# JackShDr/InfluentialRS

Hardware: AMD Instinct MI355X
Metric: scored user-item pairs/sec (whole node) (higher is better)
Workload: dtype f32; 1 GPU; c2: n_item=3415, d=128, L=200, H=4, layers=6, ffn=256; one greedy path-search step; users_per_gpu=4096, top_k=100, sweep=bf16 filter + exact f32 re-score, parallelism=single GPU

## Files before the change

influentialrs_amd/csrc/decoder.hip:

```cpp
#include "irs_internal.h"

typedef __attribute__((ext_vector_type(16))) float f32x16;

__global__ void __launch_bounds__(256) k_embed(const int64_t *__restrict__ seq, const float *__restrict__ E,
                                               const float *__restrict__ pe, float *__restrict__ x, int rows, int L,
                                               int d, float sqrtd, int64_t n_item) {
    int row = blockIdx.x * 4 + (threadIdx.x >> 6);
    int lane = threadIdx.x & 63;
    if (row >= rows) return;
    int64_t id = seq[row];
    if (id < 0) id = 0;
    if (id > n_item) id = n_item;
    int t = row % L;
    const float *e = E + id * (int64_t)d;
    const float *p = pe + (int64_t)t * d;
    float *o = x + (int64_t)row * d;
    for (int c = lane; c < d; c += 64) o[c] = __fadd_rn(__fmul_rn(e[c], sqrtd), p[c]);
}

__global__ void k_pif(const int64_t *__restrict__ user, const float *__restrict__ U, const float *__restrict__ w,
                      const float *__restrict__ b, float *__restrict__ r_u, int B, int ud, int64_t n_user) {
    int i = blockIdx.x * blockDim.x + threadIdx.x;
    if (i >= B) return;
    int64_t u = user[i];
// ... 1450 lines not shown
__device__ __forceinline__ x6_u32x4 x6_rd_sync(unsigned int base) {
    x6_u32x4 v;
    asm volatile("ds_read_b128 %0, %1 offset:%2\n\ts_waitcnt lgkmcnt(0)" : "=v"(v) : "v"(base), "i"(OFF));
    return v;
}

struct SeqTarget {
    int seq;
    float k[8], v[8];
};
__device__ __forceinline__ unsigned int seq_diag_mask(int L, int qb, bool tgt, int pq) {
    unsigned int pm = 0;
    const int k0_ = 16 * qb;
    if (L <= k0_) return 0;
    if (L - k0_ < 16) pm = (0xFFFFu << (L - k0_)) & 0xFFFFu;
    if (tgt && L - 1 >= k0_ && L - 1 < k0_ + 16) pm |= 1u << (L - 1 - k0_);
    if (pq >= k0_ && pq < k0_ + 16) pm |= 1u << (pq - k0_);
    return pm;
}
__device__ __forceinline__ void seq_attn_block(const float *Ks, const char *Vp, int PL, int L, int qb, unsigned int pm_diag, float tgt_add,
                                               bool tgt_ok, int pq, const float *qscr, float4 *of, bool store, int seq, SeqTarget &tg);
#define SEQ_KQ_SCALE 1.0f
#ifndef SEQ_ASM_DMA
#define SEQ_ASM_DMA 1
#endif
#ifndef SEQ_EXP
#define SEQ_EXP 0
#endif
#ifndef SEQ_IDLE_SKIP
#define SEQ_IDLE_SKIP 1
#endif
#ifndef SEQ_FRONT_RIDE
#define SEQ_FRONT_RIDE 1
#endif
#define X6_SEQ_VECS (256 + 12 * 32 * 4 + 384)
#define X6_SEQ_KIMG (3 * 16384 + X6_SEQ_VECS * 4)
#define X6_SEQ_VIMG (X6_SEQ_KIMG + 32768)
#define X6_SEQ_SCR (X6_SEQ_VIMG + 32768)
#define X6_SEQ_SCR_B 4608
__host__ __device__ constexpr int x6_seq_lds_bytes() { return X6_SEQ_SCR + 8 * X6_SEQ_SCR_B; }
#ifdef X6_STAMP
#define X6_T(v_) { unsigned long long t_; asm volatile("s_memtime %0\n\ts_waitcnt lgkmcnt(0)" : "=s"(t_) :: "memory"); v_ = t_; }
#if X6_STAMP + 0 == 2
#define X6_TI(v_)
#else
#define X6_TI(v_) X6_T(v_)
#endif
#define X6_PH(i_) { unsigned long long t_; asm volatile("s_memtime %0\n\ts_waitcnt lgkmcnt(0)" : "=s"(t_) :: "memory"); st_ph[i_] += t_ - st_prev; st_prev = t_; }
#else
#define X6_T(v_)
#define X6_TI(v_)
#define X6_PH(i_)
#endif
template <int QP0, int NW, bool EMBED, int NT = 4, int NPL = 3, bool SEQ = false>
__global__ void __launch_bounds__(64 * NW, (NT == 8 || NW == 8) ? 1 : 2) k_block_x6(BlockX6Args a) {
    static_assert(!SEQ || (NT == 4 && NPL == 2 && NW == 8 && !EMBED && QP0 == 3), "the sequence-resident form: d = 128, float16 planes, eight waves, no q | k | v tail");
    constexpr int NP = 8 * NPL, STEP_B = x6_step_b(NPL);
    using x6_plane = typename std::conditional<NPL == 2, x6_f16x8, x6_bf16x8>::type;
    constexpr int D = 32 * NT, F = 256, NSLOT = SEQ ? 3 : x6_nslot(NPL), LEAD = NSLOT - 1, PPW = NP / NW, HT = NT / 4;
    constexpr int NFRONT = SEQ ? 3 * NT : 0;
    constexpr float WS = x6_wscale(NPL), IWS = 1.0f / WS;
    constexpr bool RESID_LATE = X6_RESID_LATE && NPL == 2 && NT == 4 && !EMBED && NSLOT == 4 && (NW == 4 || NW == 8);
    constexpr bool RESID_SEP = RESID_LATE || SEQ;
    constexpr int NLOAD = 4 * NT;
    constexpr int NPRE = x6_npre(NT), NOUT = NT * HT;
    constexpr int S0 = EMBED ? NPRE : 0;
// ... 95 lines not shown
            for (int i = tid; i < D; i += 64 * NW) {
                vecs[V_B2 + i] = a.b2[i];
                vecs[V_G + i] = a.g[i];
                vecs[V_B + i] = a.b[i];
                vecs[V_O + 0 * D + i] = a.bo ? a.bo[i] : 0.f;
                vecs[V_O + 1 * D + i] = a.g1[i];
                vecs[V_O + 2 * D + i] = a.b1n[i];
                vecs[V_O + 3 * D + i] = a.c ? a.c[i] : 0.f;
                vecs[V_O + 4 * D + i] = a.c ? a.g2[i] : 0.f;
                vecs[V_O + 5 * D + i] = a.c ? a.b2n[i] : 0.f;
            }
        }
    }
#ifdef X6_STAGGER
    if (blockIdx.x >= 256 && blockIdx.x < 512)
        for (int i = 0; i < X6_STAGGER; ++i) __builtin_amdgcn_s_sleep(127);
#endif
    int mtile = SEQ ? (int)blockIdx.x * NW + wave : (m0 >> 5) + wave;
    const bool l_h1 = li >= 16;
    const int l_b = l_h1 ? sh_b[1] : sh_b[0];
    const int s_j = l_b >= 0 ? 16 * (l_h1 ? sh_qb[1] : sh_qb[0]) + (li & 15) : 0x3FFFFFFF;
    const int l_row0 = l_h1 ? sh_row0[1] : sh_row0[0];
    const int mt = SEQ ? 0x7FFFFFFF : m0 + wave * 32 + li;
    size_t fbase = (size_t)mtile * (4 * NT) * 64 + lane;
    const unsigned int lds0 = (unsigned int)(size_t)(__attribute__((address_space(3))) char *)smem;
    unsigned int fr_addr = lds0 + lane * 16;
    unsigned int vecs_addr = lds0 + NSLOT * STEP_B + 16 * lk;
    constexpr int qoff = NOUT * QP0;
    constexpr int nsteps_c = NFRONT + x6_nstep(NT) - qoff;
    constexpr int SEQ_LSTEPS = NFRONT + NPRE + 1;
    static_assert(!SEQ || SEQ_LSTEPS % NSLOT == 0, "slot numbering repeats per layer");
    int ly = 0, nsteps_rt = nsteps_c;
    bool last_rt = true;
#define nsteps (SEQ ? nsteps_rt : nsteps_c)
#define last (!SEQ || last_rt)
    constexpr int PPG = PPW <= 6 ? PPW : (PPW % 6 == 0 ? 6 : 4), NGRP = PPW / PPG;
    static_assert(PPW * NW == NP && PPG * NGRP == PPW, "a step's pieces divide over the waves and their issue groups");
    const uint4 *dma_src = (SEQ ? a.Wbase : a.Wx) + (PPW * wave + PPG / 2) * 64 + lane;
    const uint4 *dma_src_q = SEQ ? a.Wbase + (long long)(a.nl_total - 1) * a.wstride + (PPW * wave + PPG / 2) * 64 + lane : dma_src;
    const uint4 *dma_src_qn = dma_src;
    auto front_blk = [](int i) __attribute__((always_inline)) { return NPRE + NT * ((i % 3 + (SEQ_FRONT_RIDE ? 1 : 0)) % 3) + i / 3; };
    auto issue = [&](int i) __attribute__((always_inline)) {
        const int ib = i - NFRONT;
        int blk = (SEQ && i < NFRONT) ? front_blk(i) : (ib < NPRE ? ib : ib + qoff);
        const uint4 *dsrc = (SEQ && i < NFRONT) ? dma_src_q : dma_src;
        if (SEQ && ib >= NPRE && !last) {
            if (i == SEQ_LSTEPS - 1) return;
            blk = front_blk(i - SEQ_LSTEPS);
            dsrc = dma_src_qn;
        }
        x6_static_for<0, NGRP>([&](auto gc) __attribute__((always_inline)) {
            constexpr int grp = decltype(gc)::value;
            const uint4 *src = dsrc + (size_t)blk * (STEP_B / 16) + grp * PPG * 64;
            char *dst = smem + (i % NSLOT) * STEP_B + (PPW * wave + grp * PPG + PPG / 2) * 1024;
            if constexpr (SEQ && SEQ_ASM_DMA) {
                const unsigned int m0v = lds0 + (unsigned int)((i % NSLOT) * STEP_B + (PPW * wave + grp * PPG + PPG / 2) * 1024);
                x6_static_for<0, PPG>([&](auto jc) __attribute__((always_inline)) {
                    constexpr int off = (decltype(jc)::value - PPG / 2) * 1024;
                    const uint4 *src_ = src;
                    const unsigned int m0_ = m0v;
                    if constexpr (decltype(jc)::value == 0)
                        asm volatile("s_mov_b32 m0, %1\n\ts_nop 0\n\tglobal_load_lds_dwordx4 %0, off offset:%2" :: "v"(src_), "s"(m0_), "n"(off) : "memory", "m0");
                    else
                        asm volatile("global_load_lds_dwordx4 %0, off offset:%1" :: "v"(src_), "n"(off) : "memory");
                });
            } else {
            x6_static_for<0, PPG>([&](auto jc) __attribute__((always_inline)) {
                constexpr int off = (decltype(jc)::value - PPG / 2) * 1024;
                __builtin_amdgcn_global_load_lds((const __attribute__((address_space(1))) void *)src,
                                                 (__attribute__((address_space(3))) void *)dst, 16, off, 0);
            });
            }
        });
    };
    if constexpr (SEQ && SEQ_IDLE_SKIP) {
        if (sh_b[0] < 0 && sh_b[1] < 0) {
            issue(S0);
            asm volatile("s_waitcnt vmcnt(0) lgkmcnt(0)" ::: "memory");
            __builtin_amdgcn_s_barrier();
            x6_static_for<1, LEAD>([&](auto ic) __attribute__((always_inline)) { issue(S0 + decltype(ic)::value); });
            static_assert(LEAD == 2 && S0 == 0, "the waits below are vmcnt(0): X6_PUBLISH with three ring slots");
#pragma unroll 1
            for (ly = 0; ly <= a.n_lay; ++ly) {
                last_rt = ly == a.n_lay;
                nsteps_rt = last_rt ? NFRONT : (1 << 20);
                dma_src = a.Wbase + (long long)ly * a.wstride + (PPW * wave + PPG / 2) * 64 + lane;
                dma_src_q = a.Wbase + (long long)(ly == 0 ? a.nl_total - 1 : ly - 1) * a.wstride + (PPW * wave + PPG / 2) * 64 + lane;
                dma_src_qn = dma_src;
                float nvi[(X6_SEQ_VECS + 64 * NW - 1) / (64 * NW)];
                if (!last_rt) {
#pragma unroll
                    for (int k = 0; k < (X6_SEQ_VECS + 64 * NW - 1) / (64 * NW); ++k)
                        nvi[k] = (tid + 64 * NW * k < X6_SEQ_VECS) ? a.vecpack[(size_t)(ly + 1) * X6_SEQ_VECS + tid + 64 * NW * k] : 0.f;
                }
                x6_static_for<0, NFRONT>([&](auto ic) __attribute__((always_inline)) {
                    constexpr int i = decltype(ic)::value;
                    if (i + 1 < nsteps_rt) {
                        asm volatile("s_waitcnt vmcnt(0)" ::: "memory");
                        __builtin_amdgcn_s_barrier();
                        if (i + LEAD < nsteps_rt) issue(i + LEAD);
                    }
                    if constexpr (i % 3 == 2) __builtin_amdgcn_s_barrier();
                });
                if (last_rt) break;
                x6_static_for<NFRONT, NFRONT + NPRE>([&](auto ic) __attribute__((always_inline)) {
                    constexpr int i = decltype(ic)::value;
                    asm volatile("s_waitcnt vmcnt(0)" ::: "memory");
                    __builtin_amdgcn_s_barrier();
                    issue(i + LEAD);
                });
                asm volatile("s_waitcnt vmcnt(0)" ::: "memory");
                __builtin_amdgcn_s_barrier();
                asm volatile("" ::: "memory");
#pragma unroll
                for (int k = 0; k < (X6_SEQ_VECS + 64 * NW - 1) / (64 * NW); ++k)
                    if (tid + 64 * NW * k < X6_SEQ_VECS) vecs[tid + 64 * NW * k] = nvi[k];
                asm volatile("s_waitcnt lgkmcnt(0)" ::: "memory");
                issue(SEQ_LSTEPS - 1 + LEAD);
            }
            asm volatile("s_waitcnt vmcnt(0)" ::: "memory");
            return;
        }
    }
    f32x16 acc[NT];
    f32x16 at[NT];
    x6_u32x4 resq[RESID_SEP ? NT : 1][4];
    x6_u32x4 atq[RESID_SEP ? NT : 1][4];
    if constexpr (!EMBED) {
        const float4 *rfrag = reinterpret_cast<const float4 *>(a.Rf) + fbase;
        const float4 *afrag = reinterpret_cast<const float4 *>(a.Af) + fbase;
        if constexpr (RESID_LATE) {
            asm volatile("" ::: "memory");
            x6_static_for<0, LEAD>([&](auto ic) __attribute__((always_inline)) { issue(S0 + decltype(ic)::value); });
            asm volatile("" ::: "memory");
        }
        if constexpr (SEQ) {
            const bool live = l_b >= 0 && s_j < (l_h1 ? sh_cnt[1] : sh_cnt[0]);
            const int orig = live ? a.tok_row[(l_h1 ? sh_off[1] : sh_off[0]) + s_j] : 0;
            int64_t id = live ? a.seq[orig] : 0;
            id = id < 0 ? 0 : (id > a.n_item ? a.n_item : id);
            const float *e_ = a.E + id * (int64_t)D + 4 * lk;
            const float *p_ = a.pe + (int64_t)(orig % a.L) * D + 4 * lk;
            float4 *xw = reinterpret_cast<float4 *>(const_cast<float *>(a.Rf)) + fbase;
// ... 134 lines not shown
#define X6_MFMA(Wreg, Xp, T_) X6_MM(__builtin_bit_cast(x6_plane, Wreg), X[Xp], T_)
#ifdef X6_DUMP
#define X6_DUMP_FRAG(I_, f_) if (blockIdx.x == 0 && wave == 0) a.dbg[((I_) * NP + (f_)) * 64 + lane] = __builtin_bit_cast(uint4, af[(f_) & RA]);
#else
#define X6_DUMP_FRAG(I_, f_)
#endif
#ifdef X6_NO_READS
#define X6_READ_AHEAD(f_) asm volatile("" : "+v"(af[(f_) & RA]));
#else
#define X6_READ_AHEAD(f_)                                                                                                \
    if constexpr ((f_) + RA < NP) af[((f_) + RA) & RA] = x6_rd<((f_) + RA) * 1024>(sb_);                                 \
    else if (SEQ && !(SEQ_EXP & 2) && seq_sync_tail(step_)) af[((f_) + RA) & RA] = x6_rd_sync<((f_) + RA - NP) * 1024>(sn_);  \
    else af[((f_) + RA) & RA] = x6_rd<((f_) + RA - NP) * 1024>(sn_);  \
    asm volatile("s_waitcnt lgkmcnt(%1)" : "+v"(af[(f_) & RA]) : "i"(RA));                                               \
    X6_DUMP_FRAG(step_, f_)
#endif
#ifdef X6_NO_DMA
#define X6_ISSUE(i_)
#else
#define X6_ISSUE(i_) issue(i_)
#endif
#ifdef X6_NO_BARRIER
#define X6_PUBLISH(I_) if ((I_) + LEAD < nsteps) X6_ISSUE((I_) + LEAD);
#else
#define X6_PUBLISH(I_)                                                                                                   \
    if ((I_) + 1 < nsteps) {                                                                                             \
        X6_TI(st_a)                                                                                                       \
        if (RESID_LATE && (I_) < 4) asm volatile("s_waitcnt vmcnt(%0)" :: "i"(PPW * (LEAD - 2) + NLOAD) : "memory");  \
        else if (LEAD > 2 && (I_) + 2 < nsteps) asm volatile("s_waitcnt vmcnt(%0)" :: "i"(PPW * (LEAD - 2)) : "memory");      \
        else asm volatile("s_waitcnt vmcnt(0)" ::: "memory");                                                            \
        X6_TI(st_b)                                                                                                       \
        __builtin_amdgcn_s_barrier();                                                                                    \
        X6_TI(st_c)                                                                                                       \
        if ((I_) + LEAD < nsteps && !(SEQ && !SEQ_ASM_DMA && (I_) < NFRONT && (I_) % 3 == 2)) X6_ISSUE((I_) + LEAD);  \
        if constexpr (RESID_LATE) { if ((I_) == 1) load_res(); }                                                         \
        X6_TI(st_d)                                                                                                       \
        st_wait += st_b - st_a, st_bar += st_c - st_b, st_iss += st_d - st_c;                                            \
        if (SEQ && (I_) < NFRONT && (I_) % 3 == 0) st_ph[10] += st_c - st_b;  \
        if (SEQ && (I_) == NFRONT) st_ph[11] += st_c - st_b;                  \
    }
#endif
#define X6_STEP(I_, SRC, T0, T1, T2, T3)                                                                                \
    {                                                                                                                    \
        const int step_ = (I_);                                                                                          \
        unsigned long long sq_0 = 0, sq_1 = 0;                                                                           \
        X6_TI(sq_0)                                                                                                       \
        const unsigned int sb_ = fr_addr + (unsigned int)((step_ % NSLOT) * STEP_B);                                     \
        const unsigned int sn_ = fr_addr + (unsigned int)(((step_ + 1) % NSLOT) * STEP_B);                               \
        x6_static_for<0, NP>([&](auto fc_) __attribute__((always_inline)) {                                              \
            constexpr int f_ = decltype(fc_)::value, g_ = f_ / NPL, pl_ = f_ % NPL;                                      \
            if constexpr (f_ == 0) x6_split(SRC, 0, X);                                                                  \
            if constexpr (f_ == NP / 2) {                                                                                \
                X6_PUBLISH(step_)                                                                                        \
                x6_split(SRC, 1, X);                                                                                     \
            }                                                                                                            \
            X6_READ_AHEAD(f_)                                                                                            \
            f32x16 &T_ = (g_ & 3) == 0 ? T0 : (g_ & 3) == 1 ? T1 : (g_ & 3) == 2 ? T2 : T3;                              \
             \
            x6_static_for<0, NPL - pl_>([&](auto qc_) __attribute__((always_inline)) {                                   \
                X6_MFMA(af[f_ & RA], NPL - 1 - pl_ - decltype(qc_)::value, T_);                                           \
            });                                                                                                          \
        });                                                                                                              \
        X6_TI(sq_1)                                                                                                       \
        st_steps += sq_1 - sq_0;                                                                                         \
        __builtin_amdgcn_sched_barrier(0);                                                                               \
    }

// ... 148 lines not shown
            } else {                                                                                                     \
                constexpr int g_ = v_ - NP;                                                                              \
                X6_MM(w_, XP_[g_ >> 1][g_ & 1][0], T_);                                                                  \
            }                                                                                                            \
        });                                                                                                              \
        if constexpr (SPLIT_ACC) {                                                                                       \
            _Pragma("unroll") for (int r_ = 0; r_ < 16; ++r_) T_[r_] += ts_[r_];                                         \
        }                                                                                                                \
        X6_TI(sq_1)                                                                                                       \
        st_steps += sq_1 - sq_0;                                                                                         \
        __builtin_amdgcn_sched_barrier(0);                                                                               \
    }
    x6_plane Yp[NT][2][NPL];
    if constexpr (SEQ) {
#pragma unroll
        for (int tn = 0; tn < NT; ++tn)
#pragma unroll
            for (int s2 = 0; s2 < 2; ++s2) {
                x6_split(acc[tn], s2, Yp[tn][s2]);
                __builtin_amdgcn_sched_barrier(0);
            }
    }
    float nv[SEQ ? (X6_SEQ_VECS + 64 * NW - 1) / (64 * NW) : 1];
    unsigned long long st_q0 = 0, st_q1 = 0, st_qst = 0;
    unsigned long long st_ph[12] = {0, 0, 0, 0, 0, 0, 0, 0, 0, 0, 0, 0}, st_prev = 0;
    X6_T(st_prev)
    auto layer_body = [&]() __attribute__((always_inline)) {
    if constexpr (SEQ) {
        {
            unsigned int fb_lo = (unsigned int)fbase, fb_hi = (unsigned int)(fbase >> 32);
            asm volatile("" : "+v"(vecs_addr), "+v"(fr_addr), "+v"(mtile), "+v"(fb_lo), "+v"(fb_hi));
            fbase = ((size_t)fb_hi << 32) | fb_lo;
        }
        last_rt = ly == a.n_lay;
        nsteps_rt = last_rt ? NFRONT : (1 << 20);
        dma_src = a.Wbase + (long long)ly * a.wstride + (PPW * wave + PPG / 2) * 64 + lane;
        dma_src_q = a.Wbase + (long long)(ly == 0 ? a.nl_total - 1 : ly - 1) * a.wstride + (PPW * wave + PPG / 2) * 64 + lane;
        dma_src_qn = dma_src;
    }
    if constexpr (SEQ) {
        float *Kimg = reinterpret_cast<float *>(smem + X6_SEQ_KIMG);
        char *Vimg = smem + X6_SEQ_VIMG;
        float *scr = reinterpret_cast<float *>(smem + X6_SEQ_SCR + wave * X6_SEQ_SCR_B);
        int irow = l_row0 + s_j, li_l = li, sj_l = s_j;
        asm volatile("" : "+v"(irow), "+v"(li_l), "+v"(sj_l));
        const bool irn_ = a.mask_mode == IRS_MASK_IRN;
        float4 *ao4 = reinterpret_cast<float4 *>(const_cast<float *>(a.Af)) + (size_t)mtile * NT * 4 * 64;
#pragma unroll
        for (int h = 0; h < NT; ++h) {
            f32x16 tq, tk, tv, bt;
#pragma unroll
            for (int r = 0; r < 16; ++r) tq[r] = 0.f, tk[r] = 0.f, tv[r] = 0.f;
#if SEQ_FRONT_RIDE
            x6_u32x4 rb;
            auto front_ride = [&](auto vc, auto cc, const f32x16 &t) __attribute__((always_inline)) {
                constexpr int v = decltype(vc)::value, c = decltype(cc)::value, g = v / 6;
                static_assert(NV == 24 && RA == 3, "a bias group every six reads, used three reads behind its own read");
                typedef __attribute__((ext_vector_type(4))) _Float16 f16x4;
                if constexpr (v % 6 == 0) rb = x6_rd<32 * g>(vecs_addr + (unsigned int)((V_BQ + c * D + 32 * h) * 4));
                if constexpr (v % 6 == 3) {
#ifdef X6_NO_READS
                    asm volatile("s_waitcnt lgkmcnt(0)" : "+v"(rb));
#else
                    asm volatile("s_waitcnt lgkmcnt(%1)" : "+v"(rb) : "i"(RA));
#endif
                    const float4 bb = __builtin_bit_cast(float4, rb);
                    const float bv[4] = {bb.x, bb.y, bb.z, bb.w};
                    f16x4 hp, lp;
// ... 69 lines not shown
                }
            }
            bias_tile(bt, V_BQ + 2 * D + 32 * h);
            if (l_b >= 0) {
                typedef __attribute__((ext_vector_type(4))) _Float16 f16x4;
                const int swv = ((s_j >> 2) & 1) << 1;
#pragma unroll
                for (int g = 0; g < 4; ++g) {
                    f16x4 hp, lp;
#pragma unroll
                    for (int e = 0; e < 4; ++e) {
                        const float v = __builtin_fmaf(tv[4 * g + e], IWS, bt[4 * g + e]);
                        const _Float16 hv = (_Float16)v;
                        hp[e] = hv;
                        lp[e] = (_Float16)(v - (float)hv);
                    }
                    char *slot = Vimg + irow * 64 + ((g ^ swv) << 4) + 8 * lk;
                    *reinterpret_cast<f16x4 *>(slot) = hp;
                    *reinterpret_cast<f16x4 *>(slot + 16384) = lp;
                }
            }
#endif
            asm volatile("s_waitcnt lgkmcnt(0)" ::: "memory");
            X6_PH(0)
            __builtin_amdgcn_s_barrier();
            asm volatile("" ::: "memory");
            X6_PH(1)
            if (!(SEQ_EXP & 1)) {
                SeqTarget tg;
                tg.seq = -1;
#pragma unroll 1
                for (int blk = 0; blk < 2; ++blk) {
                    const int b_ = blk ? sh_b[1] : sh_b[0], qb_ = blk ? sh_qb[1] : sh_qb[0], row0_ = blk ? sh_row0[1] : sh_row0[0];
                    if (b_ >= 0 && last_rt && qb_ != (blk ? sh_pb[1] : sh_pb[0])) continue;
                    seq_attn_block(Kimg + row0_ * 32, Vimg + row0_ * 64, 16384, b_ >= 0 ? (blk ? sh_cnt[1] : sh_cnt[0]) : 0, b_ >= 0 ? qb_ : 16,
                                   blk ? sh_pm[1] : sh_pm[0], blk ? sh_tadd[1] : sh_tadd[0], blk ? sh_tgt[1] : sh_tgt[0],
                                   blk ? sh_pq[1] : sh_pq[0], scr + 16 * blk * 36, ao4 + (size_t)h * 4 * 64 + 16 * blk, true, b_, tg);
                }
            }
            asm volatile("" ::: "memory");
            X6_PH(2)
            if (!SEQ_ASM_DMA && 3 * h + 2 + LEAD < nsteps) issue(3 * h + 2 + LEAD);
        }
        if (last_rt) return;
        __builtin_amdgcn_fence(__ATOMIC_SEQ_CST, "workgroup");
        {
            const float4 *afrag = reinterpret_cast<const float4 *>(a.Af) + fbase;
            x6_static_for<0, NT>([&](auto tc) __attribute__((always_inline)) {
                constexpr int tn = decltype(tc)::value;
                const float4 *tp = afrag + tn * 4 * 64;
                atq[tn][0] = x6_gld<0>(tp), atq[tn][1] = x6_gld<1024>(tp), atq[tn][2] = x6_gld<2048>(tp), atq[tn][3] = x6_gld<3072>(tp);
            });
            load_res();
            static_assert(NT == 4, "sixteen operands per statement");
            asm volatile("s_waitcnt vmcnt(0)"
                         : "+v"(atq[0][0]), "+v"(atq[0][1]), "+v"(atq[0][2]), "+v"(atq[0][3]), "+v"(atq[1][0]), "+v"(atq[1][1]), "+v"(atq[1][2]),
                           "+v"(atq[1][3]), "+v"(atq[2][0]), "+v"(atq[2][1]), "+v"(atq[2][2]), "+v"(atq[2][3]), "+v"(atq[3][0]), "+v"(atq[3][1]),
                           "+v"(atq[3][2]), "+v"(atq[3][3]));
            asm volatile("" : "+v"(resq[0][0]), "+v"(resq[0][1]), "+v"(resq[0][2]), "+v"(resq[0][3]), "+v"(resq[1][0]), "+v"(resq[1][1]),
                              "+v"(resq[1][2]), "+v"(resq[1][3]), "+v"(resq[2][0]), "+v"(resq[2][1]), "+v"(resq[2][2]), "+v"(resq[2][3]),
                              "+v"(resq[3][0]), "+v"(resq[3][1]), "+v"(resq[3][2]), "+v"(resq[3][3]));
#pragma unroll
            for (int tn = 0; tn < NT; ++tn)
#pragma unroll
                for (int g = 0; g < 4; ++g) {
                    const float4 u4 = __builtin_bit_cast(float4, atq[tn][g]);
                    at[tn][4 * g + 0] = u4.x, at[tn][4 * g + 1] = u4.y, at[tn][4 * g + 2] = u4.z, at[tn][4 * g + 3] = u4.w;
#pragma unroll
                    for (int e = 0; e < 4; ++e) acc[tn][4 * g + e] = 0.f;
                }
        }
        X6_PH(3)
    }
    if constexpr (!EMBED) {
#pragma unroll
        for (int t = 0; t < NT; ++t) {
            if constexpr (RESID_LATE) {
// ... 105 lines not shown
            vec_stream(std::integral_constant<int, 2>{}, std::integral_constant<int, V_G>{}, std::integral_constant<int, V_B>{}, x6_ic0{},
                       [&](auto gc, const float4 gg, const float4 be, const float4) __attribute__((always_inline)) {
                constexpr int tn = decltype(gc)::value >> 2, g = decltype(gc)::value & 3;
                const float4 o = make_float4((acc[tn][4 * g + 0] - mu) * rstd * gg.x + be.x, (acc[tn][4 * g + 1] - mu) * rstd * gg.y + be.y,
                                             (acc[tn][4 * g + 2] - mu) * rstd * gg.z + be.z, (acc[tn][4 * g + 3] - mu) * rstd * gg.w + be.w);
                if (a.Xf) reinterpret_cast<float4 *>(a.Xf)[((size_t)(mtile * NT + tn) * 4 + g) * 64 + lane] = o;
                acc[tn][4 * g + 0] = o.x, acc[tn][4 * g + 1] = o.y, acc[tn][4 * g + 2] = o.z, acc[tn][4 * g + 3] = o.w;
            });
        } else {
#pragma unroll
        for (int tn = 0; tn < NT; ++tn)
#pragma unroll
            for (int g = 0; g < 4; ++g) {
                const int n = tn * 32 + 8 * g + 4 * lk;
                const float4 gg = *reinterpret_cast<const float4 *>(vecs + V_G + n);
                const float4 be = *reinterpret_cast<const float4 *>(vecs + V_B + n);
                const float4 o = make_float4((acc[tn][4 * g + 0] - mu) * rstd * gg.x + be.x, (acc[tn][4 * g + 1] - mu) * rstd * gg.y + be.y,
                                             (acc[tn][4 * g + 2] - mu) * rstd * gg.z + be.z, (acc[tn][4 * g + 3] - mu) * rstd * gg.w + be.w);
                if (a.Xf) reinterpret_cast<float4 *>(a.Xf)[((size_t)(mtile * NT + tn) * 4 + g) * 64 + lane] = o;
                acc[tn][4 * g + 0] = o.x, acc[tn][4 * g + 1] = o.y, acc[tn][4 * g + 2] = o.z, acc[tn][4 * g + 3] = o.w;
                __builtin_amdgcn_sched_barrier(0);
            }
        }
    }
#pragma unroll
    for (int tn = 0; tn < NT; ++tn)
#pragma unroll
        for (int s2 = 0; s2 < 2; ++s2) {
            x6_split(acc[tn], s2, Yp[tn][s2]);
            __builtin_amdgcn_sched_barrier(0);
        }
    X6_T(st_p[4])
    X6_PH(7)
    if (SEQ && !last) {
        asm volatile("s_waitcnt vmcnt(0)" ::: "memory");
        __builtin_amdgcn_s_barrier();
        asm volatile("" ::: "memory");
#pragma unroll
        for (int k = 0; k < (X6_SEQ_VECS + 64 * NW - 1) / (64 * NW); ++k)
            if (tid + 64 * NW * k < X6_SEQ_VECS) vecs[tid + 64 * NW * k] = nv[k];
        asm volatile("s_waitcnt lgkmcnt(0)" ::: "memory");
        issue(SEQ_LSTEPS - 1 + LEAD);
        af[0] = x6_rd_sync<0>(fr_addr), af[1] = x6_rd_sync<1024>(fr_addr), af[2] = x6_rd_sync<2048>(fr_addr);
        X6_PH(8)
        return;
    }
#pragma unroll
    for (int pp = 0; pp < 3; ++pp) {
        if (pp >= 3 - QP0) break;
        const int c0 = D * (pp + QP0);
#pragma unroll
        for (int i = 0; i < NT; ++i) {
            f32x16 qt, bt;
#pragma unroll
            for (int r = 0; r < 16; ++r) qt[r] = 0.f;
            X6_STEP1(NFRONT + NPRE + HT * (NT * pp + i), Yp, qt)
            if constexpr (HT == 2) { X6_STEP1(NPRE + 2 * (NT * pp + i) + 1, (&Yp[4]), qt) }
            bias_tile(bt, V_BIN + c0 + i * 32);
            X6_T(st_q0)
#ifdef X6_NO_QKV_STORE
            asm volatile("" :: "v"(qt[0]), "v"(qt[5]), "v"(qt[10]), "v"(qt[15]), "v"(bt[0]));
            if (mt < M && a.M < 0) {
#else
            if (mt < M) {
#endif
                float *qrow = a.QKV + (int64_t)mt * (3 * D) + c0 + i * 32 + 4 * lk;
                if (QP0 == 0 && a.kv_planes && pp == 2) {
                    typedef __attribute__((ext_vector_type(4))) _Float16 f16x4;
                    char *slot = reinterpret_cast<char *>(a.QKV + (int64_t)mt * (3 * D) + c0 + i * 32) + 8 * lk;
#pragma unroll
                    for (int g = 0; g < 4; ++g) {
                        f16x4 hp, lp;
#pragma unroll
                        for (int e = 0; e < 4; ++e) {
                            const float v = __builtin_fmaf(qt[4 * g + e], IWS, bt[4 * g + e]);
                            const _Float16 hv = (_Float16)v;
                            hp[e] = hv;
                            lp[e] = (_Float16)(v - (float)hv);
                        }
                        *reinterpret_cast<f16x4 *>(slot + 16 * g) = hp;
                        *reinterpret_cast<f16x4 *>(slot + 64 + 16 * g) = lp;
                    }
                } else {
#pragma unroll
                    for (int g = 0; g < 4; ++g)
                        *reinterpret_cast<float4 *>(qrow + 8 * g) =
                            make_float4(__builtin_fmaf(qt[4 * g + 0], IWS, bt[4 * g + 0]), __builtin_fmaf(qt[4 * g + 1], IWS, bt[4 * g + 1]),
                                        __builtin_fmaf(qt[4 * g + 2], IWS, bt[4 * g + 2]), __builtin_fmaf(qt[4 * g + 3], IWS, bt[4 * g + 3]));
                }
            }
            X6_T(st_q1)
            st_qst += st_q1 - st_q0;
        }
    }
    };
    if constexpr (SEQ) {
#pragma unroll 1
        for (ly = 0; ly <= a.n_lay; ++ly) layer_body();
    } else
        layer_body();
    landed_all();
#ifdef X6_STAMP
    X6_T(st_1)
    if (lane == 0 && a.stamps) {
        unsigned long long *o = a.stamps + (size_t)(blockIdx.x * NW + wave) * (SEQ ? 24 : 8);
        if constexpr (SEQ) {
#pragma unroll
            for (int i = 0; i < 12; ++i) o[8 + i] = st_ph[i];
        }
        o[0] = st_1 - st_p[0], o[1] = st_wait, o[2] = st_bar, o[3] = st_iss, o[4] = st_steps;
        o[5] = st_0 - st_p[0];
        o[6] = (st_p[2] - st_p[1]) + (st_p[4] - st_p[3]);
        o[7] = st_qst;
    }
#endif
    (void)st_ph, (void)st_prev;
    (void)st_p, (void)st_q0, (void)st_q1, (void)st_qst;
    (void)st_a, (void)st_b, (void)st_c, (void)st_d, (void)st_wait, (void)st_bar, (void)st_iss, (void)st_0, (void)st_1, (void)st_steps;
#undef nsteps
#undef last
#undef X6_STEP
#undef X6_STEP1
#undef X6_STEP1R
#undef X6_RD_V
#undef X6_WAIT_V
#undef X6_PUBLISH
#undef X6_ISSUE
#undef X6_READ_AHEAD
#undef X6_MFMA
#undef X6_MM
}

struct EmbedQkvArgs {
    const int64_t *seq;
// ... 2224 lines not shown
    }
    mx = lanes_max<56>(mx);
    if (lane == 0) red[wave][32] = mx;
    __syncthreads();
    mx = fmaxf(fmaxf(red[0][32], red[1][32]), fmaxf(red[2][32], red[3][32]));
    float sum = 0.f;
    float4 o4 = make_float4(0.f, 0.f, 0.f, 0.f);
#pragma unroll
    for (int it = 0; it < NIT; ++it) {
        const float pv = (sc[it] == -INFINITY) ? 0.f : __expf(sc[it] - mx);
        sum += pv;
        o4.x = __fmaf_rn(pv, vv[it].x, o4.x);
        o4.y = __fmaf_rn(pv, vv[it].y, o4.y);
        o4.z = __fmaf_rn(pv, vv[it].z, o4.z);
        o4.w = __fmaf_rn(pv, vv[it].w, o4.w);
    }
    sum = lanes_sum<56>(sum);
    o4.x = lanes_sum<56>(o4.x);
    o4.y = lanes_sum<56>(o4.y);
    o4.z = lanes_sum<56>(o4.z);
    o4.w = lanes_sum<56>(o4.w);
    if (lane < 8) {
        red[wave][4 * c4 + 0] = o4.x, red[wave][4 * c4 + 1] = o4.y, red[wave][4 * c4 + 2] = o4.z, red[wave][4 * c4 + 3] = o4.w;
        if (lane == 0) red[wave][33] = sum;
    }
    __syncthreads();
    if (tid < HD) {
        const float o = red[0][tid] + red[1][tid] + red[2][tid] + red[3][tid];
        const float l = red[0][33] + red[1][33] + red[2][33] + red[3][33];
        out_rows[(int64_t)b * d + h * HD + tid] = o / l;
    }
}

__global__ void __launch_bounds__(256) k_ln(const float *__restrict__ z, const float *__restrict__ g1,
                                            const float *__restrict__ b1, const float *__restrict__ c,
                                            const float *__restrict__ g2, const float *__restrict__ b2,
                                            float *__restrict__ y, int rows, int d, const int32_t *__restrict__ m_dev) {
    int row = blockIdx.x * 4 + (threadIdx.x >> 6);
    int lane = threadIdx.x & 63;
    if (row >= rows || (m_dev && row >= m_dev[0])) return;
    const float *zr = z + (int64_t)row * d;
    float v[8];
    float s = 0.f;
#pragma unroll
    for (int i = 0; i < 8; ++i) {
        int col = lane + 64 * i;
        v[i] = (col < d) ? zr[col] : 0.f;
        s += v[i];
    }
    const float invd = 1.0f / (float)d;
    float mu = wave_sum(s) * invd;
    float q = 0.f;
#pragma unroll
    for (int i = 0; i < 8; ++i) {
        int col = lane + 64 * i;
        float t = (col < d) ? v[i] - mu : 0.f;
        q += t * t;
    }
    float rstd = 1.0f / sqrtf(wave_sum(q) * invd + 1e-5f);
#pragma unroll
    for (int i = 0; i < 8; ++i) {
        int col = lane + 64 * i;
        if (col < d) v[i] = (v[i] - mu) * rstd * g1[col] + b1[col];
    }
    if (c) {
        s = 0.f;
// ... 673 lines not shown
    case DecFam::SMALL16:
    case DecFam::WIDE:
    case DecFam::ANY: {
        SmallBlockArgs sb = small_args(ctx, r.layer, l, ctx->act_ao, x, nullptr, y, qkv_buf(c, l + 1), c.rows, c.m_dev,
                                       l + 1 < ctx->dims.n_layers);
        if (r.att_fused) {
            sb.QKVin = qkv_buf(c, l), sb.r_u = ctx->act_ru, sb.seq_last = c.seq + (ctx->dims.max_len - 1), sb.cnt = c.cnt;
            sb.padq = ctx->seq_padq, sb.mask_mode = ctx->dims.mask_mode;
        }
        launch_small(ctx, r.layer, sb, r.att_fused, c.rows > SMALL_MT2_ROWS, c.s);
        c.x = y;
        c.y = x;
        return IRS_OK;
    }
    default:
        return gemm_rest(ctx, r.layer == DecFam::GEMM_LN, l, ctx->act_ao, x, r.layer == DecFam::GEMM_LN ? y : x, y, x, c.rows, c.m_dev,
                         c.s);
    }
}

static int last_layer(const DecodeCall &c, int l, const int32_t *pos, float *xrows) {
    irs_ctx *ctx = c.ctx;
    const DecodeRoute &r = c.r;
    const int L = ctx->dims.max_len, d = ctx->dims.d, H = ctx->dims.n_heads, B = c.B;
    const irs_layer_w &w = ctx->layer[l];
    const int32_t *qrow = c.qrow;
    const hipStream_t s = c.s;
    int rc;
    float *xf = ctx->act_xf, *h_r = ctx->act_h;
    float *ao_r = ctx->act_ao, *x_r = ao_r + (size_t)B * d, *y_r = ao_r + (size_t)2 * B * d, *z_r = ao_r + (size_t)3 * B * d;
    const float *q_r = nullptr;
    const int nt = d > 128 ? d / 32 : 4;
    if (r.seq) {
        hipLaunchKernelGGL(k_gather_rows_frag, dim3(B), dim3(64), 0, s, xf, ctx->qrow_tile, x_r, d, nt);
        hipLaunchKernelGGL(k_gather_rows_frag, dim3(B), dim3(64), 0, s, ctx->act_yf, ctx->qrow_tile, ao_r, d, nt);
    } else if (r.kv_only) {
        hipLaunchKernelGGL(k_gather_rows_frag, dim3(B), dim3(64), 0, s, xf, qrow, x_r, d, nt);
        LinArgs q{};
        q.X = x_r, q.W = w.sa_in_w, q.bias = w.sa_in_b, q.Y = h_r, q.M = B, q.N = d, q.K = d;
        if ((rc = launch_linear(ctx, q, s))) return rc;
        q_r = h_r;
    }
    irs_prof_begin(ctx, IRS_PROF_ATTN, s);
    if (r.seq) {
    } else if (d / H == 32 && L <= 256 && d % 4 == 0 && (((uintptr_t)ctx->act_qkv | (uintptr_t)q_r) & 15) == 0)
        hipLaunchKernelGGL(k_attn_row32, dim3(H, B), dim3(256), 0, s, ctx->act_qkv, c.seq, ctx->act_ru, ao_r, L, d,
                           ctx->dims.mask_mode, c.off, c.cnt, qrow, q_r, ctx->seq_padq);
    else
        hipLaunchKernelGGL(k_attn_row, dim3(H, B), dim3(64), 0, s, ctx->act_qkv, c.seq, ctx->act_ru, pos, ao_r, L, d, d / H,
                           ctx->dims.mask_mode, c.off, c.cnt, c.tok, qrow, q_r);
    irs_prof_end(ctx, IRS_PROF_ATTN, s, 4.0 * B * (double)L * d, 4.0 * 3.0 * B * (double)L * d);
    const bool small = r.tail == DecFam::SMALL16 || r.tail == DecFam::WIDE || r.tail == DecFam::ANY;
    const bool idx_res = small && !r.frag;
    if (r.frag && !r.kv_only) hipLaunchKernelGGL(k_gather_rows_frag, dim3(B), dim3(64), 0, s, xf, qrow, x_r, d, nt);
    else if (!r.frag && !idx_res) hipLaunchKernelGGL(k_gather_rows_idx, dim3(B), dim3(64), 0, s, c.x, qrow, x_r, d);
    if (small) {
        const SmallBlockArgs sb = small_args(ctx, r.tail, l, ao_r, idx_res ? c.x : x_r, idx_res ? qrow : nullptr, xrows, nullptr, B,
                                             nullptr, false);
        launch_small(ctx, r.tail, sb, false, B > 2048, s);
    } else if ((rc = gemm_rest(ctx, r.tail == DecFam::GEMM_LN, l, ao_r, x_r, y_r, z_r, xrows, B, nullptr, s))) {
        return rc;
    }
    IRS_CHECK_HIP(ctx, hipGetLastError());
    return IRS_OK;
}

int irs_launch_decode(irs_ctx *ctx, const int64_t *seq, const int64_t *user, int B, float *x_out, const int32_t *pos,
                      float *xrows, float *r_u_out, hipStream_t s) {
// ... 52 lines not shown
```

Measured before the change: 2.260 billion pairs/s.

## Absorb last-layer attention into query-side projections instead of full-sequence KV pass

The fused sequence kernel now stops one layer early, so the final layer's K/V projection for every position is no longer computed. Three new kernels handle that layer for the query row only. They fold W_q·x into a per-head vector u = W_k^T q plus a bias term, run the masked softmax attention directly over the raw layer inputs x, and then apply W_v and its bias to the attention-weighted sums. This trades the full-sequence K/V GEMM and attention for per-user matrix-vector work, and relies on softmax weights summing to one to move the V bias outside. The added risk is that masking and target-slot semantics must match the fused path exactly.

```diff
diff --git a/influentialrs_amd/csrc/decoder.hip b/influentialrs_amd/csrc/decoder.hip
--- a/influentialrs_amd/csrc/decoder.hip
+++ b/influentialrs_amd/csrc/decoder.hip
@@ -1506,6 +1506,9 @@
 #endif
 #ifndef SEQ_FRONT_RIDE
 #define SEQ_FRONT_RIDE 1
+#endif
+#ifndef SEQ_LAST_ABSORB
+#define SEQ_LAST_ABSORB 1
 #endif
 #define X6_SEQ_VECS (256 + 12 * 32 * 4 + 384)
 #define X6_SEQ_KIMG (3 * 16384 + X6_SEQ_VECS * 4)
@@ -1667,8 +1670,9 @@
     static_assert(!SEQ || SEQ_LSTEPS % NSLOT == 0, "slot numbering repeats per layer");
     int ly = 0, nsteps_rt = nsteps_c;
     bool last_rt = true;
-#define nsteps (SEQ ? nsteps_rt : nsteps_c)
-#define last (!SEQ || last_rt)
+    bool end_rt = false;
+#define nsteps (SEQ ? (SEQ_LAST_ABSORB ? (1 << 20) : nsteps_rt) : nsteps_c)
+#define last (!SEQ || (!SEQ_LAST_ABSORB && last_rt))
     constexpr int PPG = PPW <= 6 ? PPW : (PPW % 6 == 0 ? 6 : 4), NGRP = PPW / PPG;
     static_assert(PPW * NW == NP && PPG * NGRP == PPW, "a step's pieces divide over the waves and their issue groups");
     const uint4 *dma_src = (SEQ ? a.Wbase : a.Wx) + (PPW * wave + PPG / 2) * 64 + lane;
@@ -1716,34 +1720,39 @@
             x6_static_for<1, LEAD>([&](auto ic) __attribute__((always_inline)) { issue(S0 + decltype(ic)::value); });
             static_assert(LEAD == 2 && S0 == 0, "the waits below are vmcnt(0): X6_PUBLISH with three ring slots");
 #pragma unroll 1
-            for (ly = 0; ly <= a.n_lay; ++ly) {
+            for (ly = 0; ly < a.n_lay + (SEQ_LAST_ABSORB ? 0 : 1); ++ly) {
+#if SEQ_LAST_ABSORB
+                end_rt = ly == a.n_lay - 1;
+#else
                 last_rt = ly == a.n_lay;
                 nsteps_rt = last_rt ? NFRONT : (1 << 20);
+#endif
                 dma_src = a.Wbase + (long long)ly * a.wstride + (PPW * wave + PPG / 2) * 64 + lane;
                 dma_src_q = a.Wbase + (long long)(ly == 0 ? a.nl_total - 1 : ly - 1) * a.wstride + (PPW * wave + PPG / 2) * 64 + lane;
                 dma_src_qn = dma_src;
                 float nvi[(X6_SEQ_VECS + 64 * NW - 1) / (64 * NW)];
-                if (!last_rt) {
+                if (!last && !end_rt) {
 #pragma unroll
                     for (int k = 0; k < (X6_SEQ_VECS + 64 * NW - 1) / (64 * NW); ++k)
                         nvi[k] = (tid + 64 * NW * k < X6_SEQ_VECS) ? a.vecpack[(size_t)(ly + 1) * X6_SEQ_VECS + tid + 64 * NW * k] : 0.f;
                 }
                 x6_static_for<0, NFRONT>([&](auto ic) __attribute__((always_inline)) {
                     constexpr int i = decltype(ic)::value;
-                    if (i + 1 < nsteps_rt) {
+                    if (i + 1 < nsteps) {
                         asm volatile("s_waitcnt vmcnt(0)" ::: "memory");
                         __builtin_amdgcn_s_barrier();
-                        if (i + LEAD < nsteps_rt) issue(i + LEAD);
+                        if (i + LEAD < nsteps) issue(i + LEAD);
                     }
                     if constexpr (i % 3 == 2) __builtin_amdgcn_s_barrier();
                 });
-                if (last_rt) break;
+                if (last) break;
                 x6_static_for<NFRONT, NFRONT + NPRE>([&](auto ic) __attribute__((always_inline)) {
                     constexpr int i = decltype(ic)::value;
                     asm volatile("s_waitcnt vmcnt(0)" ::: "memory");
                     __builtin_amdgcn_s_barrier();
-                    issue(i + LEAD);
+                    if (!(i == NFRONT + NPRE - 1 && end_rt)) issue(i + LEAD);
                 });
+                if (end_rt) break;
                 asm volatile("s_waitcnt vmcnt(0)" ::: "memory");
                 __builtin_amdgcn_s_barrier();
                 asm volatile("" ::: "memory");
@@ -1944,7 +1953,9 @@
         X6_TI(st_b)                                                                                                       \
         __builtin_amdgcn_s_barrier();                                                                                    \
         X6_TI(st_c)                                                                                                       \
-        if ((I_) + LEAD < nsteps && !(SEQ && !SEQ_ASM_DMA && (I_) < NFRONT && (I_) % 3 == 2)) X6_ISSUE((I_) + LEAD);  \
+        if ((I_) + LEAD < nsteps && !(SEQ && !SEQ_ASM_DMA && (I_) < NFRONT && (I_) % 3 == 2) &&                          \
+            !(SEQ && SEQ_LAST_ABSORB && (I_) == NFRONT + NPRE - 1 && end_rt))  \
+            X6_ISSUE((I_) + LEAD);  \
         if constexpr (RESID_LATE) { if ((I_) == 1) load_res(); }                                                         \
         X6_TI(st_d)                                                                                                       \
         st_wait += st_b - st_a, st_bar += st_c - st_b, st_iss += st_d - st_c;                                            \
@@ -2159,8 +2170,12 @@
             asm volatile("" : "+v"(vecs_addr), "+v"(fr_addr), "+v"(mtile), "+v"(fb_lo), "+v"(fb_hi));
             fbase = ((size_t)fb_hi << 32) | fb_lo;
         }
+#if SEQ_LAST_ABSORB
+        end_rt = ly == a.n_lay - 1;
+#else
         last_rt = ly == a.n_lay;
         nsteps_rt = last_rt ? NFRONT : (1 << 20);
+#endif
         dma_src = a.Wbase + (long long)ly * a.wstride + (PPW * wave + PPG / 2) * 64 + lane;
         dma_src_q = a.Wbase + (long long)(ly == 0 ? a.nl_total - 1 : ly - 1) * a.wstride + (PPW * wave + PPG / 2) * 64 + lane;
         dma_src_qn = dma_src;
@@ -2296,7 +2311,7 @@
 #pragma unroll 1
                 for (int blk = 0; blk < 2; ++blk) {
                     const int b_ = blk ? sh_b[1] : sh_b[0], qb_ = blk ? sh_qb[1] : sh_qb[0], row0_ = blk ? sh_row0[1] : sh_row0[0];
-                    if (b_ >= 0 && last_rt && qb_ != (blk ? sh_pb[1] : sh_pb[0])) continue;
+                    if (b_ >= 0 && last && qb_ != (blk ? sh_pb[1] : sh_pb[0])) continue;
                     seq_attn_block(Kimg + row0_ * 32, Vimg + row0_ * 64, 16384, b_ >= 0 ? (blk ? sh_cnt[1] : sh_cnt[0]) : 0, b_ >= 0 ? qb_ : 16,
                                    blk ? sh_pm[1] : sh_pm[0], blk ? sh_tadd[1] : sh_tadd[0], blk ? sh_tgt[1] : sh_tgt[0],
                                    blk ? sh_pq[1] : sh_pq[0], scr + 16 * blk * 36, ao4 + (size_t)h * 4 * 64 + 16 * blk, true, b_, tg);
@@ -2306,7 +2321,7 @@
             X6_PH(2)
             if (!SEQ_ASM_DMA && 3 * h + 2 + LEAD < nsteps) issue(3 * h + 2 + LEAD);
         }
-        if (last_rt) return;
+        if (last) return;
         __builtin_amdgcn_fence(__ATOMIC_SEQ_CST, "workgroup");
         {
             const float4 *afrag = reinterpret_cast<const float4 *>(a.Af) + fbase;
@@ -2478,6 +2493,7 @@
         }
     X6_T(st_p[4])
     X6_PH(7)
+    if (SEQ && SEQ_LAST_ABSORB && end_rt) return;
     if (SEQ && !last) {
         asm volatile("s_waitcnt vmcnt(0)" ::: "memory");
         __builtin_amdgcn_s_barrier();
@@ -2542,10 +2558,11 @@
     };
     if constexpr (SEQ) {
 #pragma unroll 1
-        for (ly = 0; ly <= a.n_lay; ++ly) layer_body();
+        for (ly = 0; ly < a.n_lay + (SEQ_LAST_ABSORB ? 0 : 1); ++ly) layer_body();
     } else
         layer_body();
     landed_all();
+    if constexpr (SEQ && SEQ_LAST_ABSORB) asm volatile("s_waitcnt vmcnt(0)" ::: "memory");
 #ifdef X6_STAMP
     X6_T(st_1)
     if (lane == 0 && a.stamps) {
@@ -4836,6 +4853,237 @@
     }
 }
 
+#define ABS_SQ 8
+#define ABS_SO 8
+#define ABS_WLD 132
+__device__ __forceinline__ void absorb_stage64(const float *__restrict__ W, int r0, float *Ws, int tid) {
+#pragma unroll
+    for (int k = 0; k < 8; ++k) {
+        const int idx = tid + 256 * k, row = idx >> 5, c4 = idx & 31;
+        *reinterpret_cast<float4 *>(Ws + row * ABS_WLD + 4 * c4) = *reinterpret_cast<const float4 *>(W + (size_t)(r0 + row) * 128 + 4 * c4);
+    }
+}
+__global__ void __launch_bounds__(256) k_absorb_qu(const float *__restrict__ xf, const int32_t *__restrict__ qrow_tile,
+                                                   const float *__restrict__ Win, const float *__restrict__ bin, float *__restrict__ x_r,
+                                                   float *__restrict__ u, float *__restrict__ cq, int B) {
+    constexpr int D = 128, HD = 32, S = ABS_SQ;
+    __shared__ __attribute__((aligned(16))) float Ws[64 * ABS_WLD];
+    __shared__ __attribute__((aligned(16))) float xs[S][D], qs[S][D];
+    const int tid = threadIdx.x, b0 = blockIdx.x * S;
+#pragma unroll
+    for (int k = 0; k < S * D / 256; ++k) {
+        const int idx = tid + 256 * k, s = idx >> 7, c = idx & 127, b = b0 + s;
+        float v = 0.f;
+        if (b < B) {
+            const int row = qrow_tile[b];
+            v = xf[(((size_t)(row >> 5) * 4 + (c >> 5)) * 4 + ((c >> 3) & 3)) * 256 + ((c >> 2) & 1) * 128 + (row & 31) * 4 + (c & 3)];
+            x_r[(size_t)b * D + c] = v;
+        }
+        xs[s][c] = v;
+    }
+    const float scale = 1.0f / sqrtf((float)HD);
+    {
+        const int r = tid & 63, sg = tid >> 6;
+        const float *wp = Win + (size_t)(tid >> 5) * D + 4 * (tid & 31);
+        float *wl = Ws + (tid >> 5) * ABS_WLD + 4 * (tid & 31);
+        const float4 wa0 = *reinterpret_cast<const float4 *>(wp + 0 * 8 * D), wa1 = *reinterpret_cast<const float4 *>(wp + 1 * 8 * D),
+                     wa2 = *reinterpret_cast<const float4 *>(wp + 2 * 8 * D), wa3 = *reinterpret_cast<const float4 *>(wp + 3 * 8 * D),
+                     wa4 = *reinterpret_cast<const float4 *>(wp + 4 * 8 * D), wa5 = *reinterpret_cast<const float4 *>(wp + 5 * 8 * D),
+                     wa6 = *reinterpret_cast<const float4 *>(wp + 6 * 8 * D), wa7 = *reinterpret_cast<const float4 *>(wp + 7 * 8 * D);
+        const float4 wb0 = *reinterpret_cast<const float4 *>(wp + 8 * 8 * D), wb1 = *reinterpret_cast<const float4 *>(wp + 9 * 8 * D),
+                     wb2 = *reinterpret_cast<const float4 *>(wp + 10 * 8 * D), wb3 = *reinterpret_cast<const float4 *>(wp + 11 * 8 * D),
+                     wb4 = *reinterpret_cast<const float4 *>(wp + 12 * 8 * D), wb5 = *reinterpret_cast<const float4 *>(wp + 13 * 8 * D),
+                     wb6 = *reinterpret_cast<const float4 *>(wp + 14 * 8 * D), wb7 = *reinterpret_cast<const float4 *>(wp + 15 * 8 * D);
+#pragma unroll
+        for (int ch = 0; ch < 2; ++ch) {
+            __syncthreads();
+#define ABS_ST(k_, a_, b_) *reinterpret_cast<float4 *>(wl + (k_) * 8 * ABS_WLD) = ch == 0 ? a_ : b_
+            ABS_ST(0, wa0, wb0), ABS_ST(1, wa1, wb1), ABS_ST(2, wa2, wb2), ABS_ST(3, wa3, wb3);
+            ABS_ST(4, wa4, wb4), ABS_ST(5, wa5, wb5), ABS_ST(6, wa6, wb6), ABS_ST(7, wa7, wb7);
+#undef ABS_ST
+            __syncthreads();
+            const float bq = bin[64 * ch + r];
+            float acc[2] = {bq, bq};
+#pragma unroll 8
+            for (int k4 = 0; k4 < D / 4; ++k4) {
+                const float4 w = *reinterpret_cast<const float4 *>(Ws + r * ABS_WLD + 4 * k4);
+#pragma unroll
+                for (int s = 0; s < 2; ++s) {
+                    const float4 x4 = *reinterpret_cast<const float4 *>(&xs[2 * sg + s][4 * k4]);
+                    acc[s] = __fmaf_rn(w.x, x4.x, acc[s]);
+                    acc[s] = __fmaf_rn(w.y, x4.y, acc[s]);
+                    acc[s] = __fmaf_rn(w.z, x4.z, acc[s]);
+                    acc[s] = __fmaf_rn(w.w, x4.w, acc[s]);
+                }
+            }
+#pragma unroll
+            for (int s = 0; s < 2; ++s) qs[2 * sg + s][64 * ch + r] = acc[s] * scale;
+        }
+    }
+    __syncthreads();
+    {
+        const int k = tid & 127, hf = tid >> 7;
+#pragma unroll 1
+        for (int h = 0; h < 4; ++h) {
+            float acc[4] = {0.f, 0.f, 0.f, 0.f};
+#pragma unroll 16
+            for (int c = 0; c < HD; ++c) {
+                const float w = Win[(size_t)(D + h * HD + c) * D + k];
+#pragma unroll
+                for (int s = 0; s < 4; ++s) acc[s] = __fmaf_rn(w, qs[4 * hf + s][h * HD + c], acc[s]);
+            }
+#pragma unroll
+            for (int s = 0; s < 4; ++s)
+                if (b0 + 4 * hf + s < B) u[((size_t)(b0 + 4 * hf + s) * 4 + h) * D + k] = acc[s];
+        }
+    }
+    if (tid < 4 * S) {
+        const int s = tid >> 2, h = tid & 3;
+        float acc = 0.f;
+        for (int c = 0; c < HD; ++c) acc = __fmaf_rn(qs[s][h * HD + c], bin[D + h * HD + c], acc);
+        if (b0 + s < B) cq[(size_t)(b0 + s) * 4 + h] = acc;
+    }
+}
+
+__global__ void __launch_bounds__(256) k_absorb_attn(const float *__restrict__ xf, float *__restrict__ um, const float *__restrict__ cq,
+                                                     const int64_t *__restrict__ seq, const float *__restrict__ r_u, int Lmax,
+                                                     int mask_mode, const int32_t *__restrict__ off, const int32_t *__restrict__ cnt,
+                                                     const int32_t *__restrict__ qrow, const int32_t *__restrict__ padq,
+                                                     const int32_t *__restrict__ row0, const int32_t *__restrict__ qrow_tile) {
+    __shared__ __attribute__((aligned(16))) float xs[2][16 * 128];
+    const int b = blockIdx.x, tid = threadIdx.x, lane = tid & 63, h = tid >> 6, r = lane & 15, q = lane >> 4;
+    const int L = cnt[b];
+    int i = qrow[b] - off[b];
+    if (i < 0) i = 0;
+    if (i >= L) i = L - 1;
+    int T = (L + 15) >> 4;
+    T = T < 1 ? 1 : (T > SEQ_WG_BLOCKS ? SEQ_WG_BLOCKS : T);
+    const int slot = row0[b] >> 4;
+    const int h0 = (qrow_tile[b] >> 8) * (2 * SEQ_WG_TILES) + slot;
+    const bool irn = mask_mode == IRS_MASK_IRN;
+    const bool has_tgt = seq[(int64_t)b * Lmax + Lmax - 1] != 0;
+    const float add_allowed = irn ? r_u[b] : 0.f;
+    const int pq = padq[b];
+    const int ib = i >> 4;
+    const bool tgt_blk = irn && has_tgt && T - 1 > ib;
+    const int nblk = ib + 1 + (tgt_blk ? 1 : 0);
+    float *umh = um + ((size_t)b * 4 + h) * 128;
+    float4 u4[8];
+#pragma unroll
+    for (int k = 0; k < 8; ++k) u4[k] = *reinterpret_cast<const float4 *>(umh + 16 * k + 4 * q);
+    const float ch = cq[(size_t)b * 4 + h];
+    auto blk_of = [&](int n) { return n <= ib ? n : T - 1; };
+    auto gload = [&](float4 (&g)[2], int blk) __attribute__((always_inline)) {
+        const int hidx = h0 + seq_half_of_block(slot & 1, T, blk);
+        const float *p = xf + (size_t)(hidx >> 1) * 4096 + (hidx & 1) * 64 + (tid >> 4) * 128 + (tid & 15) * 4;
+        const bool live = 16 * blk + (tid & 15) < L;
+#pragma unroll
+        for (int kk = 0; kk < 2; ++kk) g[kk] = live ? *reinterpret_cast<const float4 *>(p + 2048 * kk) : make_float4(0.f, 0.f, 0.f, 0.f);
+    };
+    auto sstore = [&](int buf, const float4 (&g)[2]) __attribute__((always_inline)) {
+#pragma unroll
+        for (int kk = 0; kk < 2; ++kk) *reinterpret_cast<float4 *>(&xs[buf][4 * (tid + 256 * kk)]) = g[kk];
+    };
+    float acc[32];
+#pragma unroll
+    for (int c = 0; c < 32; ++c) acc[c] = 0.f;
+    float mrun = -INFINITY, lsum = 0.f;
+    float4 g[2];
+    gload(g, blk_of(0));
+    sstore(0, g);
+    if (nblk > 1) gload(g, blk_of(1));
+    __syncthreads();
+#pragma unroll 1
+    for (int n = 0; n < nblk; ++n) {
+        const float *xb = &xs[n & 1][4 * (16 * q + r)];
+        float4 x[8];
+#pragma unroll
+        for (int k = 0; k < 8; ++k) x[k] = *reinterpret_cast<const float4 *>(xb + 256 * k);
+        const int j = 16 * blk_of(n) + r;
+        const bool is_tgt = irn && has_tgt && j == L - 1;
+        const bool ok = j < L && j != pq && (is_tgt || j <= i);
+        float s = 0.f;
+#pragma unroll
+        for (int k = 0; k < 8; ++k) {
+            s = __fmaf_rn(u4[k].x, x[k].x, s);
+            s = __fmaf_rn(u4[k].y, x[k].y, s);
+            s = __fmaf_rn(u4[k].z, x[k].z, s);
+            s = __fmaf_rn(u4[k].w, x[k].w, s);
+        }
+        s = lanes_sum<48>(s);
+        const float sc = ok ? (s + ch) + (is_tgt ? 1.0f : add_allowed) : -INFINITY;
+        const float mnew = fmaxf(mrun, lanes_max<15>(sc));
+        if (mnew != mrun) {
+            const float al = mrun == -INFINITY ? 1.0f : __expf(mrun - mnew);
+            lsum *= al;
+#pragma unroll
+            for (int c = 0; c < 32; ++c) acc[c] *= al;
+            mrun = mnew;
+        }
+        const float p = sc == -INFINITY ? 0.f : __expf(sc - mnew);
+        lsum += p;
+#pragma unroll
+        for (int k = 0; k < 8; ++k) {
+            acc[4 * k + 0] = __fmaf_rn(p, x[k].x, acc[4 * k + 0]);
+            acc[4 * k + 1] = __fmaf_rn(p, x[k].y, acc[4 * k + 1]);
+            acc[4 * k + 2] = __fmaf_rn(p, x[k].z, acc[4 * k + 2]);
+            acc[4 * k + 3] = __fmaf_rn(p, x[k].w, acc[4 * k + 3]);
+        }
+        if (n + 1 < nblk) {
+            sstore((n + 1) & 1, g);
+            if (n + 2 < nblk) gload(g, blk_of(n + 2));
+        }
+        __syncthreads();
+    }
+    const float l = lanes_sum<15>(lsum);
+#pragma unroll
+    for (int k = 0; k < 8; ++k) {
+        const float4 o = make_float4(lanes_sum<15>(acc[4 * k + 0]), lanes_sum<15>(acc[4 * k + 1]), lanes_sum<15>(acc[4 * k + 2]),
+                                     lanes_sum<15>(acc[4 * k + 3]));
+        if (r == k) *reinterpret_cast<float4 *>(umh + 16 * k + 4 * q) = make_float4(o.x / l, o.y / l, o.z / l, o.w / l);
+    }
+}
+
+__global__ void __launch_bounds__(256) k_absorb_out(const float *__restrict__ m, const float *__restrict__ Win, const float *__restrict__ bin,
+                                                    float *__restrict__ ao_r, int B) {
+    constexpr int D = 128, S = ABS_SO;
+    __shared__ __attribute__((aligned(16))) float Ws[64 * ABS_WLD];
+    __shared__ __attribute__((aligned(16))) float ms[S][4 * D];
+    const int tid = threadIdx.x, b0 = blockIdx.x * S;
+#pragma unroll
+    for (int k = 0; k < S * 4 * D / 4 / 256; ++k) {
+        const int idx = tid + 256 * k, s = idx >> 7, c4 = idx & 127;
+        float4 v = make_float4(0.f, 0.f, 0.f, 0.f);
+        if (b0 + s < B) v = *reinterpret_cast<const float4 *>(m + (size_t)(b0 + s) * 4 * D + 4 * c4);
+        *reinterpret_cast<float4 *>(&ms[s][4 * c4]) = v;
+    }
+    const int r = tid & 63, sg = tid >> 6;
+#pragma unroll 1
+    for (int ch = 0; ch < 2; ++ch) {
+        __syncthreads();
+        absorb_stage64(Win, 2 * D + 64 * ch, Ws, tid);
+        __syncthreads();
+        const int row = 64 * ch + r, h = row >> 5;
+        const float bv = bin[2 * D + row];
+        float acc[2] = {bv, bv};
+#pragma unroll 4
+        for (int k4 = 0; k4 < D / 4; ++k4) {
+            const float4 w = *reinterpret_cast<const float4 *>(Ws + r * ABS_WLD + 4 * k4);
+#pragma unroll
+            for (int s = 0; s < 2; ++s) {
+                const float4 m4 = *reinterpret_cast<const float4 *>(&ms[2 * sg + s][h * D + 4 * k4]);
+                acc[s] = __fmaf_rn(w.x, m4.x, acc[s]);
+                acc[s] = __fmaf_rn(w.y, m4.y, acc[s]);
+                acc[s] = __fmaf_rn(w.z, m4.z, acc[s]);
+                acc[s] = __fmaf_rn(w.w, m4.w, acc[s]);
+            }
+        }
+#pragma unroll
+        for (int s = 0; s < 2; ++s)
+            if (b0 + 2 * sg + s < B) ao_r[(size_t)(b0 + 2 * sg + s) * D + row] = acc[s];
+    }
+}
+
 __global__ void __launch_bounds__(256) k_ln(const float *__restrict__ z, const float *__restrict__ g1,
                                             const float *__restrict__ b1, const float *__restrict__ c,
                                             const float *__restrict__ g2, const float *__restrict__ b2,
@@ -5575,8 +5823,17 @@
     const float *q_r = nullptr;
     const int nt = d > 128 ? d / 32 : 4;
     if (r.seq) {
+#if SEQ_LAST_ABSORB
+        float *um = ctx->act_h, *cq = um + (size_t)B * 4 * d;
+        hipLaunchKernelGGL(k_absorb_qu, dim3((B + ABS_SQ - 1) / ABS_SQ), dim3(256), 0, s, xf, ctx->qrow_tile, w.sa_in_w, w.sa_in_b, x_r, um,
+                           cq, B);
+        hipLaunchKernelGGL(k_absorb_attn, dim3(B), dim3(256), 0, s, xf, um, cq, c.seq, ctx->act_ru, L, ctx->dims.mask_mode, c.off, c.cnt,
+                           qrow, ctx->seq_padq, ctx->seq_row0, ctx->qrow_tile);
+        hipLaunchKernelGGL(k_absorb_out, dim3((B + ABS_SO - 1) / ABS_SO), dim3(256), 0, s, um, w.sa_in_w, w.sa_in_b, ao_r, B);
+#else
         hipLaunchKernelGGL(k_gather_rows_frag, dim3(B), dim3(64), 0, s, xf, ctx->qrow_tile, x_r, d, nt);
         hipLaunchKernelGGL(k_gather_rows_frag, dim3(B), dim3(64), 0, s, ctx->act_yf, ctx->qrow_tile, ao_r, d, nt);
+#endif
     } else if (r.kv_only) {
         hipLaunchKernelGGL(k_gather_rows_frag, dim3(B), dim3(64), 0, s, xf, qrow, x_r, d, nt);
         LinArgs q{};
```

After: 2.328 billion pairs/s (median of 6 runs). +3.0%, better.
